# anguswilliams91/bpl-next

Hardware: NVIDIA B200
Metric: logdensity_grad_match_evals_per_s (higher is better)
Workload: dtype f32

## Files before the change

bpl_next_b200/csrc/api.cu:

```cuda
#include <limits.h>
#include <stdarg.h>
#include <stdlib.h>
#include <string.h>

#include <algorithm>
#include <atomic>
#include <mutex>
#include <new>

#include "common.cuh"
#include "plan.h"
#include "problem.h"
#include "loo.h"
#include "score_grid.h"
#include "simulate.h"

namespace bplx {

static thread_local char g_err[1024] = "";
static std::atomic<unsigned long long> g_launches{0};

void set_error(const char* fmt, ...) {
  va_list ap;
  va_start(ap, fmt);
// ... 59 lines not shown
    }
#pragma unroll
  for (int s = 0; s < 4; s++)
#pragma unroll
    for (int k = 0; k < 4; k++) tile[s][threadIdx.y + 8 * k][threadIdx.x] = v[s][k];
  __syncthreads();
#pragma unroll
  for (int s = 0; s < 4; s++)
#pragma unroll
    for (int k = 0; k < 4; k++) {
      const int c = c0 + threadIdx.y + 8 * k, r = r0 + s * 32 + threadIdx.x;
      if (r < R && c < Cc) out[(size_t)c * ldo + r] = tile[s][threadIdx.x][threadIdx.y + 8 * k];
    }
}
static int launch_transpose(const float* in, float* out, int R, int Cc, size_t ldi, size_t ldo, cudaStream_t s) {
  const dim3 grid((unsigned)((Cc + 31) / 32), (unsigned)((R + 127) / 128));
  BPLX_REQUIRE(grid.y <= 65535u, BPLX_E_UNSUPPORTED, "transpose of %d rows", R);
  transpose_kernel<<<grid, dim3(32, 8), 0, s>>>(in, out, R, Cc, ldi, ldo);
  BPLX_CUDA(cudaGetLastError());
  note_launch(1);
  return BPLX_OK;
}

static size_t align256(size_t n) { return (n + 255) / 256 * 256; }
static size_t transpose_room(const KernelParams& kp, int C) {
  if ((size_t)C * (size_t)kp.D < env_switches().transpose_min_elems) return 0;
  return 2 * (((size_t)C + 31) / 32 * 32) * (size_t)kp.D * sizeof(float);
}

static size_t workspace_bytes(const KernelParams& kp, int C) {
  const size_t Cpad = ((size_t)C + 31) / 32 * 32;
  if (kp.model == BPLX_DYNAMIC)
    return ((size_t)kp.G * kp.T * 2 + (kp.dyn_hyp_ws ? (size_t)kp.G * 16 : 0)) * Cpad * sizeof(float);
  if (kp.Cf <= 0) return 0;
  return (size_t)kp.V * Cpad * sizeof(float);
}

static int enqueue(const bplx_problem* p, int C, int layout, int ld, const float* theta, float* lp, float* grad,
                   float* corr_coef, void* ws, size_t ws_bytes, cudaStream_t stream, bool pdl = false, bool lik = false) {
  BPLX_REQUIRE(p != nullptr, BPLX_E_INVALID, "problem is NULL");
  BPLX_REQUIRE(C > 0, BPLX_E_INVALID, "num_chains must be positive (got %d)", C);
  BPLX_REQUIRE(theta && lp && grad, BPLX_E_INVALID, "theta, lp and grad must not be NULL");
  if (layout == BPLX_CHAIN_MAJOR && !env_switches().no_transpose) {
    const size_t base = align256(workspace_bytes(p->kp, C)), room = transpose_room(p->kp, C);
    if (room > 0 && ws != nullptr && ws_bytes >= base + room) {
      const int Dc = lik ? p->lik_D : p->kp.D;
      const size_t ldm = ld > 0 ? (size_t)ld : (size_t)Dc, Cpad = ((size_t)C + 31) / 32 * 32;
      BPLX_REQUIRE(ldm >= (size_t)Dc, BPLX_E_INVALID, "chain-major ld (%d) < D (%d)", ld, Dc);
      float* tin = reinterpret_cast<float*>(static_cast<char*>(ws) + base);
      float* tout = tin + Cpad * (size_t)p->kp.D;
      int rc = launch_transpose(theta, tin, C, Dc, ldm, Cpad, stream);
      if (rc != BPLX_OK) return rc;
      rc = enqueue(p, C, BPLX_CHAIN_MINOR, (int)Cpad, tin, lp, tout, corr_coef, ws, base, stream, pdl, lik);
      if (rc != BPLX_OK) return rc;
      return launch_transpose(tout, grad, Dc, C, Cpad, ldm, stream);
    }
  }
  KernelParams kp = p->kp;
  if (lik) {
    BPLX_REQUIRE(kp.model != BPLX_DYNAMIC, BPLX_E_UNSUPPORTED, "bplx_loglik_fwdbwd: DYNAMIC is not supported");
    kp.lik_only = 1;
    kp.off = p->lik_off;
    for (int i = 0; i < 12; i++) kp.hyper[i] = p->lik_hyper[i];
    kp.nhyper = p->lik_nhyper;
    kp.D = p->lik_D;
    kp.K = 0;
    kp.const_term = p->lik_const;
  }
// ... 7 lines not shown
    BPLX_REQUIRE(kp.sd >= C, BPLX_E_INVALID, "chain-minor ld (%d) < num_chains (%d)", ld, C);
  } else {
    BPLX_REQUIRE(false, BPLX_E_INVALID, "unknown layout %d", layout);
  }
  BPLX_REQUIRE((long long)kp.D * (long long)kp.sd + (long long)C * (long long)kp.sc < (1ll << 31), BPLX_E_UNSUPPORTED,
               "theta / grad of %d x %d elements exceed the 31-bit element index of the kernel", C, kp.D);
  const size_t need = workspace_bytes(kp, C);
  BPLX_REQUIRE(ws_bytes >= need && (need == 0 || ws != nullptr), BPLX_E_WORKSPACE,
               "workspace too small: %zu bytes given, %zu needed", ws_bytes, need);
  kp.C = C;
  kp.Cpad = (C + 31) / 32 * 32;
  kp.theta = theta;
  kp.lp = lp;
  kp.grad = grad;
  kp.corr_coef = corr_coef;
  kp.scratch = static_cast<float*>(ws);
  int si = 0;
  const int groups = (C + kChains - 1) / kChains;
  for (int i = kNumSplits - 1; i >= 1; i--)
    if (p->s1[i] && (1 << i) <= kp.split_hint && groups <= p->max_clusters[i]) {
      si = i;
      break;
    }
  if (const int want = env_switches().split) {
    for (int i = 0; i < kNumSplits; i++)
      if ((1 << i) == want && p->s1[i] && (i == 0 || p->max_clusters[i] > 0)) si = i;
  }
  auto use_split = [&](int i) {
    kp.split = 1 << i;
    kp.stream1 = p->s1[i];
    kp.stream2 = p->s2[i];
    kp.warp_b1 = p->wb1[i];
    kp.warp_b2 = p->wb2[i];
  };
  use_split(si);
  kp.group0 = 0;
  kp.ngroups = groups;
  if (kp.model == BPLX_DYNAMIC) return launch_logdensity_dynamic(kp, stream);
  int ti = 0;
  const int rest = p->sm_count > 0 ? groups % p->sm_count : 0;
  if (si == 0 && rest > 0 && rest < groups && !env_switches().split && !env_switches().no_tail_split) {
    for (int i = kNumSplits - 1; i >= 1; i--)
      if (p->s1[i] && (1 << i) <= kp.split_hint && rest <= p->max_clusters[i] && rest * (1 << i) <= p->sm_count) {
        ti = i;
        break;
      }
  }
  if (ti == 0) return launch_logdensity(kp, p->wb[si], stream, pdl);
  kp.ngroups = groups - rest;
  int rc = launch_logdensity(kp, p->wb[0], stream, pdl);
  if (rc != BPLX_OK) return rc;
  use_split(ti);
  kp.group0 = groups - rest;
  kp.ngroups = rest;
  return launch_logdensity(kp, p->wb[ti], stream, pdl);
}

}

using namespace bplx;

extern "C" {

int bplx_problem_create(const bplx_problem_desc* desc, bplx_problem** out) {
  BPLX_REQUIRE(desc && out, BPLX_E_INVALID, "desc / out is NULL");
  *out = nullptr;
  HostPlan hp;
  std::string err;
  int rc = build_plan(*desc, &hp, &err);
  if (rc != BPLX_OK) {
    set_error("%s", err.c_str());
    return rc;
  }
  bplx_problem* p = new (std::nothrow) bplx_problem();
  BPLX_REQUIRE(p, BPLX_E_NOMEM, "out of host memory");
  auto fail = [&](int code) {
    bplx_problem_destroy(p);
    return code;
  };
  if (cudaGetDevice(&p->device) != cudaSuccess) {
    set_error("cudaGetDevice failed: no usable CUDA device (bplx has no CPU fallback)");
    return fail(BPLX_E_CUDA);
  }
  p->kp = hp.kp;
  p->layout = hp.layout;
  p->lik_off = hp.lik_off;
  for (int i = 0; i < 12; i++) p->lik_hyper[i] = hp.lik_hyper[i];
  p->lik_nhyper = hp.lik_nhyper;
  p->lik_D = hp.lik_D;
  p->lik_const = hp.lik_const;
  p->lik_layout = hp.lik_layout;
  KernelParams& kp = p->kp;
#define UP(vec, ptr)                                 \
  if ((rc = upload(p, hp.vec, &(ptr))) != BPLX_OK) return fail(rc)
  UP(stream1, p->s1[0]);
  UP(stream2, p->s2[0]);
  UP(warp_b1, p->wb1[0]);
  UP(warp_b2, p->wb2[0]);
  for (int i = 1; i < kNumSplits; i++) {
    if (hp.more[i - 1].stream1.empty()) continue;
    UP(more[i - 1].stream1, p->s1[i]);
    UP(more[i - 1].stream2, p->s2[i]);
    UP(more[i - 1].warp_b1, p->wb1[i]);
    UP(more[i - 1].warp_b2, p->wb2[i]);
  }
  auto keep_bounds = [&](int i, const std::vector<uint32_t>& b1, const std::vector<uint32_t>& b2) {
    const size_t cap = sizeof(p->wb[i].b1) / sizeof(uint32_t);
    for (size_t k = 0; k < b1.size() && k < cap; k++) p->wb[i].b1[k] = b1[k];
    for (size_t k = 0; k < b2.size() && k < cap; k++) p->wb[i].b2[k] = b2[k];
  };
  keep_bounds(0, hp.warp_b1, hp.warp_b2);
  for (int i = 1; i < kNumSplits; i++) keep_bounds(i, hp.more[i - 1].warp_b1, hp.more[i - 1].warp_b2);
  kp.stream1 = p->s1[0];
  kp.stream2 = p->s2[0];
  kp.warp_b1 = p->wb1[0];
  kp.warp_b2 = p->wb2[0];
  kp.split = 1;
  UP(team_vptr, kp.team_vptr);
  UP(team_flags, kp.team_flags);
  UP(v_team, kp.v_team);
  UP(v_conf, kp.v_conf);
  UP(conf_vptr, kp.conf_vptr);
  UP(conf_vlist, kp.conf_vlist);
  UP(yexp, kp.yexp);
  UP(yteam, kp.yteam);
  UP(yconf, kp.yconf);
  UP(Xs, kp.Xs);
  UP(gw_tptr, kp.gw_tptr);
  UP(gw_tlist, kp.gw_tlist);
#undef UP
  rc = kp.model == BPLX_DYNAMIC ? logdensity_dynamic_set_attributes() : logdensity_set_attributes(kp);
  if (rc != BPLX_OK) return fail(rc);
  if (cudaDeviceGetAttribute(&p->sm_count, cudaDevAttrMultiProcessorCount, p->device) != cudaSuccess) p->sm_count = 0;
  p->max_clusters[0] = 1 << 30;
  if (kp.model != BPLX_DYNAMIC)
    for (int i = 1; i < kNumSplits; i++) p->max_clusters[i] = p->s1[i] ? logdensity_max_clusters(kp, 1 << i) : 0;
  p->stats[0] = desc->num_matches;
  p->stats[1] = hp.n1;
  p->stats[2] = hp.n1_padded;
  p->stats[3] = hp.n2;
  p->stats[4] = hp.n2_padded;
  p->stats[5] = kp.smem_total;
  p->stats[6] = kp.nwarps;
  p->stats[7] = kp.V;
  if (kp.model != BPLX_DYNAMIC) {
    p->warp_stats.assign((size_t)kp.nwarps * 12, 0);
    for (int phase = 0; phase < 2; phase++) {
      const std::vector<unsigned char>& S = phase ? hp.stream2 : hp.stream1;
      const std::vector<uint32_t>& wb = phase ? hp.warp_b2 : hp.warp_b1;
      const size_t esz = (phase == 0 && kp.clip) ? sizeof(EntryClip) : sizeof(Entry);
      const uint32_t minp = phase ? kp.min_piece2 : kp.min_piece1;
      for (int w = 0; w < kp.nwarps && w + 1 < (int)wb.size(); w++) {
        long long* o = &p->warp_stats[(size_t)w * 12 + phase * 6];
        const uint32_t len = wb[w + 1] - wb[w];
        o[5] = (len + kp.stage_bytes - 1) / kp.stage_bytes;
        for (uint32_t st = 0; st < len; st += kp.stage_bytes) {
// ... 783 lines not shown
```

bpl_next_b200/csrc/k1_common.cuh:

```cuda
#pragma once
#include <float.h>

#include "common.cuh"
#include "plan.h"

namespace bplx {

namespace {


constexpr float kLn2 = 0.693147180559945309f;
constexpr unsigned kFull = 0xffffffffu;

struct Hyp {
  float mu_d, sig_a, sig_d, mu[4], sig[4];
};

struct Lane {
  const float* th;
  float* gr;
  float* sc;
  int sd;
  bool active;
  __device__ __forceinline__ float ld(int d) const { return __ldg(th + (uint32_t)(d * sd)); }
// ... 71 lines not shown
  if (kind == kH1) {
    g[eAh1] += gx; g[eBh1] += gy;
  } else if (kind == kA1) {
    g[eBa1] += gx; g[eAa1] += gy;
  } else {
    g[eB0] += gx; g[eA0] += gy;
  }
}

template <bool ADD>
__device__ __forceinline__ void put_raw(const KernelParams& kp, const Lane& ln, int t, const float (&g)[6], float& hacc) {
  const ThetaOffsets& o = kp.off;
  const float ra = g[eAh1] + g[eAa1] + g[eA0];
  const float rd = -(g[eBh1] + g[eBa1] + g[eB0]);
  const float rx[4] = {g[eAh1], g[eAa1], -g[eBh1], -g[eBa1]};
  if (kp.ndec == 0) hacc += rx[0];
  if (!ln.active) return;
  if (ADD) {
    red_add(ln.g(o.za + t), ra);
    red_add(ln.g(o.zd + t), rd);
  } else {
    *ln.g(o.za + t) = ra;
    *ln.g(o.zd + t) = rd;
  }
#pragma unroll
  for (int i = 0; i < 4; i++) {
    if (i < kp.ndec) {
      if (ADD) red_add(ln.g(o.dec[i] + t), rx[i]);
      else *ln.g(o.dec[i] + t) = rx[i];
    }
  }
}

__device__ __forceinline__ void put_side(const KernelParams& kp, float* q, const float (&g)[6], float& hacc) {
  q[0] = g[eAh1] + g[eAa1] + g[eA0];
  q[32] = -(g[eBh1] + g[eBa1] + g[eB0]);
  const float rx[4] = {g[eAh1], g[eAa1], -g[eBh1], -g[eBa1]};
  if (kp.ndec == 0) hacc += rx[0];
#pragma unroll
  for (int i = 0; i < 4; i++)
    if (i < kp.ndec) q[(2 + i) * 32] = rx[i];
}

struct Ring {
  uint32_t ring, bar;
  uint32_t S;
  const unsigned char* src;
  uint32_t total;
  uint32_t gs0, gs_next;
  int lane;

  __device__ __forceinline__ void init(uint32_t ring_, uint32_t bar_, uint32_t S_, int lane_) {
    ring = ring_; bar = bar_; S = S_; lane = lane_;
    total = gs0 = gs_next = 0;
    src = nullptr;
    if (lane == 0) {
#pragma unroll
      for (int s = 0; s < kStages; s++) mbar_init(bar + 8 * s, 1);
      fence_mbar_init();
      fence_proxy_async();
    }
    __syncwarp();
  }
  __device__ __forceinline__ void issue(uint32_t k) {
    const uint32_t b0 = k * S;
    if (lane == 0 && b0 < total) {
      const uint32_t bytes = min(S, total - b0);
      const uint32_t slot = (gs0 + k) % kStages;
      mbar_arrive_expect_tx(bar + 8 * slot, bytes);
      tma_load_1d(ring + slot * S, src + b0, bytes, bar + 8 * slot);
    }
  }
  __device__ __forceinline__ void begin(const void* src_, uint32_t total_bytes) {
    __syncwarp();
// ... 140 lines not shown
```

bpl_next_b200/csrc/logdensity.cu:

```cuda
#include <cooperative_groups.h>

#include <math.h>

#include "k1_common.cuh"
#include "problem.h"

namespace cg = cooperative_groups;

#ifdef BPLX_TIMELINE
__device__ unsigned long long g_timeline[32 * 24];
#define BPLX_STAMP(i)                                                                    \
  do {                                                                                   \
    if (blockIdx.x == 0 && (threadIdx.x & 31) == 0) {                                    \
      unsigned long long t_;                                                             \
      asm volatile("mov.u64 %0, %%globaltimer;" : "=l"(t_));                             \
      g_timeline[(threadIdx.x >> 5) * 24 + (i)] = t_;                                    \
    }                                                                                    \
  } while (0)
#define BPLX_STAMP_DEP(i, dep)                                                           \
  do {                                                                                   \
    if (blockIdx.x == 0 && (threadIdx.x & 31) == 0) {                                    \
      unsigned long long t_;                                                             \
      asm volatile("mov.u64 %0, %%globaltimer;" : "=l"(t_) : "f"(dep));                  \
      g_timeline[(threadIdx.x >> 5) * 24 + (i)] = t_;                                    \
// ... 397 lines not shown
  BPLX_STAMP(5);
  float gc = 0.0f;
  {
    float g[6] = {0.0f, 0.0f, 0.0f, 0.0f, 0.0f, 0.0f}, cacc = 0.0f;
    const uint32_t nst = ring.num_stages();
    for (uint32_t k = 0; k < nst; k++) {
      uint32_t bytes;
      const uint32_t a0 = ring.acquire(k, &bytes);
      if (k == 0) BPLX_STAMP(18);
      uint32_t a = a0;
      const uint32_t aend = a0 + bytes;
      while (a + kp.min_piece2 <= aend) {
        const Hdr L = unpack_hdr(lds128u(a));
        a += 16;
        if (L.flags & kTeamFirst) {
#pragma unroll
          for (int e = 0; e < 6; e++) g[e] = 0.0f;
        }
        float2 own = lds64(tab + L.own_off);
        if (L.kind >= kH0) { const float s = own.x; own.x = own.y; own.y = s; }
        const bool home = (L.kind & 1) == 0;
        float lt, du, gx, gy;
        if (!CLIP) tau_piece<kTauPlain>(a, L, own, home, cc, tab, lt, du, gx, gy);
        else if (noclip) tau_piece<kTauUnclipped>(a, L, own, home, cc, tab, lt, du, gx, gy);
        else tau_piece<kTauClipped>(a, L, own, home, cc, tab, lt, du, gx, gy);
        if (home) {
          lp_acc = fmaf(lt, kLn2, lp_acc);
          gc += du;
        }
        add_own(g, L.kind, gx, gy);
        if (kp.Cf > 0) {
          cacc += L.kind == kH1 ? gx - gy : gy - gx;
          if (L.flags & kVteamLast) {
            if (ln.active) red_add(ln.sc + (size_t)L.vteam * kp.Cpad, cacc);
            cacc = 0.0f;
          }
        }
        if (L.flags & kTeamLast) {
          if (p2s) put_side(kp, p2_tab + (((L.kind & 1) * kp.T + L.team) * (2 + ndec)) * 32 + lane, g, hacc);
          else put_raw<true>(kp, ln, (int)L.team, g, hacc);
        }
      }
      ring.release(k);
    }
  }
  BPLX_STAMP(6);
  red_gc[warp * 32 + lane] = gc;
  __syncthreads();
  gc = 0.0f;
  for (int w = 0; w < W; w++) gc += red_gc[w * 32 + lane];
  if (S > 1) {
    if (warp == 0) dsm_st_f32(a_cl + (uint32_t)(crank * 32 + lane) * 4u, gc);
    cg::this_cluster().sync();
    gc = 0.0f;
    for (int q = 0; q < S; q++) gc += dsm_ld_f32(a_cl + (uint32_t)(q * 32 + lane) * 4u);
  }
  {
    const float t11 = fmaxf(1.0f - cc, 0.0f);
    gc -= kp.w11 / t11;
    if (vwarp == 0 && kp.w11 != 0.0f) lp_acc = fmaf(kp.w11, logf(t11), lp_acc);
  }

  BPLX_STAMP(7);
  Fixup fx;
  fx.h1 = 0u;
  fx.confs = 0u;
#pragma unroll
  for (int which = 0; which < 2; which++) {
    const uint32_t packed = dsm_ld_u32(a_found + (uint32_t)(which * 32 + lane) * 4u);
    fx.teams[which] = 0xffffffffu;
    fx.vts[which] = 0xffffffffu;
    fx.vx[which] = fx.vy[which] = 0.0f;
// ... 10 lines not shown
        fx.vy[0] = (qlam == 1 && yfree) ? wgt : 0.0f;
      } else {
        const float wgt = -gc * r / best[2];
        fx.vx[1] = xfree ? wgt : 0.0f;
        fx.vy[1] = yfree ? wgt : 0.0f;
      }
      fx.h1 |= (h1 ? 1u : 0u) << which;
      fx.vts[which] = own_v | (opp_v << 16);
      if (kp.Cf > 0)
        fx.confs |= ((uint32_t)__ldg(kp.v_conf + own_v) | ((uint32_t)__ldg(kp.v_conf + opp_v) << 8)) << (16 * which);
    }
  }

  BPLX_STAMP(8);
  const bool has_rho = !dc && !lik;
  const float pri = lik ? 0.0f : 1.0f;
  float u = 0.5f, rho = 0.0f, inv_s2 = 1.0f;
  if (has_rho) {
    u = red_hyp[11 * 32 + lane];
    rho = 2.0f * u - 1.0f;
    inv_s2 = 1.0f / (1.0f - rho * rho);
  }
  float a_mu_d = 0.0f, a_ls_a = 0.0f, a_ls_d = 0.0f, a_rho = 0.0f, a_mu[4], a_ls[4];
#pragma unroll
  for (int i = 0; i < 4; i++) a_mu[i] = a_ls[i] = 0.0f;
  {
    Hyp hy;
    hy.mu_d = red_hyp[0 * 32 + lane]; hy.sig_a = red_hyp[1 * 32 + lane]; hy.sig_d = red_hyp[2 * 32 + lane];
#pragma unroll
    for (int i = 0; i < 4; i++) { hy.mu[i] = red_hyp[(3 + i) * 32 + lane]; hy.sig[i] = red_hyp[(7 + i) * 32 + lane]; }

    for (int t = vwarp; t < kp.T; t += VW) {
      const float za = ln.ld(o.za + t), zd = ln.ld(o.zd + t);
      const uint32_t v0 = (uint32_t)__ldg(kp.team_vptr + t), nv = (uint32_t)__ldg(kp.team_vptr + t + 1) - v0;
      const float4 ys = __ldg(reinterpret_cast<const float4*>(kp.yteam + (size_t)t * 8));
      const float2 ys2 = __ldg(reinterpret_cast<const float2*>(kp.yteam + (size_t)t * 8 + 4));
      float ra = ld_cg(ln.g(o.za + t)) + ys.x;
      float rd = ld_cg(ln.g(o.zd + t)) + ys.y;
      float rx[4] = {ys.z, ys.w, ys2.x, ys2.y};
      float dec[4] = {0.0f, 0.0f, 0.0f, 0.0f};
#pragma unroll
      for (int i = 0; i < 4; i++) {
        if (i < ndec) {
          dec[i] = ln.ld(o.dec[i] + t);
          rx[i] += ld_cg(ln.g(o.dec[i] + t));
        }
      }
      if (p2s) {
#pragma unroll
        for (int side = 0; side < 2; side++) {
          const float* q = p2_tab + ((side * kp.T + t) * (2 + ndec)) * 32 + lane;
          ra += q[0];
          rd += q[32];
#pragma unroll
          for (int i = 0; i < 4; i++)
            if (i < ndec) rx[i] += q[(2 + i) * 32];
        }
      }
#pragma unroll
      for (int which = 0; which < 2; which++) {
        if ((fx.vts[which] & 0xffffu) - v0 < nv) fold_fixup(fx, which, 0, ra, rd, rx);
        if ((fx.vts[which] >> 16) - v0 < nv) fold_fixup(fx, which, 1, ra, rd, rx);
      }
      float p_za, p_zd;
      if (has_rho) {
        const float e = zd - rho * za;
        const float es = e * inv_s2;
        lp_acc -= 0.5f * (za * za + e * es);
        p_za = -za + rho * es;
        p_zd = -es;
        a_rho += es * za - rho * es * es + rho * inv_s2;
      } else {
        lp_acc -= pri * 0.5f * (za * za + zd * zd);
        p_za = -pri * za;
        p_zd = -pri * zd;
      }
      if (ln.active) {
        *ln.g(o.za + t) = fmaf(hy.sig_a, ra, p_za);
        *ln.g(o.zd + t) = fmaf(hy.sig_d, rd, p_zd);
      }
      a_ls_a = fmaf(hy.sig_a * za, ra, a_ls_a);
      a_ls_d = fmaf(hy.sig_d * zd, rd, a_ls_d);
      a_mu_d += rd;
      if (dc) a_mu[0] += rx[0];
#pragma unroll
      for (int i = 0; i < 4; i++) {
        if (i < ndec) {
          lp_acc -= pri * 0.5f * dec[i] * dec[i];
          if (ln.active) *ln.g(o.dec[i] + t) = fmaf(hy.sig[i], rx[i], -pri * dec[i]);
          a_mu[i] += rx[i];
          a_ls[i] = fmaf(hy.sig[i] * dec[i], rx[i], a_ls[i]);
        }
      }
      if (kp.K > 0) {
        dsm_st_f32(a_teamrows + (uint32_t)(t * 64 + lane) * 4u, ra);
        dsm_st_f32(a_teamrows + (uint32_t)(t * 64 + 32 + lane) * 4u, rd);
      }
    }
    if (dc) a_mu[0] += hacc;
  }
  for (int k = vwarp; k < kp.Cf; k += VW) {
    const float cf = ln.ld(o.conf + k);
    float s = __ldg(kp.yconf + k) - pri * cf;
    lp_acc -= pri * 0.5f * cf * cf;
    const int j0 = __ldg(kp.conf_vptr + k), j1 = __ldg(kp.conf_vptr + k + 1);
    for (int j = j0; j < j1; j++) s += ld_cg(ln.sc + (size_t)__ldg(kp.conf_vlist + j) * kp.Cpad);
#pragma unroll
    for (int ws = 0; ws < 4; ws++)
      if (fx.vts[ws >> 1] != 0xffffffffu && ((fx.confs >> (8 * ((ws >> 1) * 2 + (ws & 1)))) & 0xffu) == (uint32_t)k)
        s += fixup_conf(fx, ws >> 1, ws & 1);
    if (ln.active) *ln.g(o.conf + k) = s;
  }

  BPLX_STAMP(9);
  float* part = reinterpret_cast<float*>(smem + kp.epi_part);
  {
    float* p = part + (size_t)warp * kPartRows * 32 + lane;
    p[0 * 32] = lp_acc; p[1 * 32] = a_mu_d; p[2 * 32] = a_ls_a; p[3 * 32] = a_ls_d;
#pragma unroll
    for (int i = 0; i < 4; i++) { p[(4 + i) * 32] = a_mu[i]; p[(8 + i) * 32] = a_ls[i]; }
    p[12 * 32] = a_rho;
  }
  __syncthreads();
  if (S > 1) {
    for (int row = warp; row < kAccRows; row += W) {
      float s = 0.0f;
      for (int w = 0; w < W; w++) s += part[((size_t)w * kPartRows + row) * 32 + lane];
      dsm_st_f32(a_partcl + (uint32_t)((crank * kPartRows + row) * 32 + lane) * 4u, s);
    }
    cg::this_cluster().sync();
    if (crank != 0) return;
  }
  BPLX_STAMP(10);
  auto total = [&](int row) {
    float s = 0.0f;
    if (S > 1) {
      for (int q = 0; q < S; q++) s += dsm_ld_f32(a_partcl + (uint32_t)((q * kPartRows + row) * 32 + lane) * 4u);
    } else {
      for (int w = 0; w < W; w++) s += part[((size_t)w * kPartRows + row) * 32 + lane];
// ... 129 lines not shown
```

bpl_next_b200/csrc/plan.cc:

```cpp
#include "plan.h"

#include <algorithm>
#include <cmath>
#include <cstdarg>
#include <cstdio>
#include <cstdlib>
#include <cstring>
#include <map>
#include <numeric>

namespace bplx {
namespace {

struct RawEntry {
  uint32_t opp;
  uint8_t cls;
  double w, wyx, wyy;
};

std::string fmt(const char* f, ...) {
  char buf[512];
  va_list ap;
  va_start(ap, f);
  vsnprintf(buf, sizeof buf, f, ap);
  va_end(ap);
  return buf;
}

void add_site(std::string* s, const char* name, int off, int count, const char* tr) {
  *s += fmt("%s:%d:%d:%s;", name, off, count, tr);
}

int make_layout(int model, int T, int K, int Cf, ThetaOffsets* o, std::string* s) {
  ThetaOffsets z;
  memset(&z, 0xff, sizeof z);
  int d = 0;
  auto scalar = [&](const char* n, const char* tr) { add_site(s, n, d, 1, tr); return d++; };
  auto vec = [&](const char* n, int cnt, const char* tr) {
    add_site(s, n, d, cnt, tr);
    int r = d;
    d += cnt;
    return r;
// ... 284 lines not shown
    for (size_t i = 0; i < yc.size(); i++) P.yconf[i] = (float)yc[i];
  }
  P.Xs.assign(d.covariates ? d.covariates : nullptr, d.covariates ? d.covariates + (size_t)T * K : nullptr);

  auto own_off = [&](int v, int kind) -> uint32_t {
    uint32_t base = kind == kH1 ? kp.tabP1 : kind == kA1 ? kp.tabQ1 : kp.tabP0;
    return base + (uint32_t)v * kRowBytes;
  };
  auto opp_base = [&](int kind) -> uint32_t { return kind == kH1 ? kp.tabQ1 : kind == kA1 ? kp.tabP1 : kp.tabP0; };

  auto merge = [](std::vector<RawEntry>& v) {
    std::stable_sort(v.begin(), v.end(), [](const RawEntry& a, const RawEntry& b) {
      return a.cls != b.cls ? a.cls < b.cls : a.opp < b.opp;
    });
    size_t o = 0;
    for (size_t i = 0; i < v.size(); i++) {
      if (o && v[o - 1].cls == v[i].cls && v[o - 1].opp == v[i].opp) {
        v[o - 1].w += v[i].w;
        v[o - 1].wyx += v[i].wyx;
        v[o - 1].wyy += v[i].wyy;
      } else {
        v[o++] = v[i];
      }
    }
    v.resize(o);
  };
  for (auto& v : raw1) merge(v);
  for (auto& v : raw2) merge(v);
  P.team_flags.assign(T, 0);
  for (int v = 0; v < V; v++)
    for (int k = 0; k < 4; k++)
      if (!raw1[(size_t)v * 4 + k].empty()) P.team_flags[P.v_team[v]] |= 1;

  auto team_costs = [&](const std::vector<std::vector<RawEntry>>& raw, double per_entry, double per_list,
                        double per_team) {
    std::vector<double> cost(T, 0.0);
    for (int v = 0; v < V; v++)
      for (int k = 0; k < 4; k++) {
        const size_t n = raw[(size_t)v * 4 + k].size();
        if (n) cost[P.v_team[v]] += per_list * (1.0 + (double)n / 100.0) + per_entry * (double)n;
      }
    for (int t = 0; t < T; t++)
      if (cost[t] > 0.0) cost[t] += per_team;
    return cost;
  };
  auto assign = [&](const std::vector<double>& cost, int W, std::vector<std::vector<int>>* teams) {
    std::vector<int> order(T);
    std::iota(order.begin(), order.end(), 0);
    std::stable_sort(order.begin(), order.end(), [&](int a, int b) { return cost[a] > cost[b]; });
    std::vector<double> load(W, 0.0);
    teams->assign(W, {});
    for (int t : order) {
      if (cost[t] == 0.0) continue;
      int best = 0;
      for (int w = 1; w < W; w++)
        if (load[w] < load[best]) best = w;
      load[best] += cost[t];
      (*teams)[best].push_back(t);
    }
    for (auto& v : *teams) std::sort(v.begin(), v.end());
    return *std::max_element(load.begin(), load.end());
  };
  const std::vector<double> cost1 = team_costs(raw1, kp.clip ? 16.0 : 6.0, 40.0, 30.0);
  const std::vector<double> cost2 = team_costs(raw2, 12.0, 60.0, 30.0);
  auto smem_need = [&](int W, uint32_t stage) {
    const uint32_t epi = (K > 0 ? (uint32_t)T * kRowBytes : 0u) + (uint32_t)(W + kMaxSplit) * kPartRows * 128u;
    const uint32_t tabb = (std::max(table_bytes, epi) + 127u) / 128u * 128u;
    return tabb + (uint32_t)W * kStages * stage + 128u + (uint32_t)W * kStages * 8u + 3u * 256u + 2u * 128u + 2u * 128u +
           12u * 128u + (uint32_t)(W + kMaxSplit) * 128u;
  };
  const uint32_t kSmemMax = 227u * 1024u;
  int W = 0;
  uint32_t stage = 1024;
  std::vector<std::vector<int>> w1, w2;
  if (force_warps <= 0) {
    if (const char* e = getenv("BPLX_NWARPS")) force_warps = atoi(e);
  }
  if (const char* e = getenv("BPLX_STAGE")) stage = (uint32_t)atoi(e) == 512u ? 512u : 1024u;
  if (force_warps > 0) {
    W = std::max(1, std::min(force_warps, kMaxWarps));
    if (smem_need(W, stage) > kSmemMax) stage = 512;
  } else {
    double best = 0.0;
    for (int cand : {4, 8, 12, 16, 20, 24}) {
      if (cand > kMaxWarps) continue;
      uint32_t st = stage;
      if (smem_need(cand, st) > kSmemMax) st = 512;
      if (smem_need(cand, st) > kSmemMax) continue;
      std::vector<std::vector<int>> t1, t2;
      const double span = assign(cost1, cand, &t1) + assign(cost2, cand, &t2) + 4.0 * cand + (st == 512 ? 0.05 * best : 0.0);
      if (W == 0 || span < 0.97 * best) best = span, W = cand, stage = st;
    }
    if (W == 0) W = 4, stage = 512;
  }
  kp.nwarps = W;
  kp.stage_bytes = stage;
  kp.force_clip_forms = 0;
  if (const char* e = getenv("BPLX_CLIP_FORMS")) kp.force_clip_forms = atoi(e);
  {
    std::vector<std::vector<int>> t1, t2;
    const double span = assign(cost1, W, &t1) + assign(cost2, W, &t2);
    kp.split_hint = span >= 32000.0 ? 8 : span >= 16000.0 ? 4 : span >= 8000.0 ? 2 : 1;
  }

  std::vector<std::vector<int>> w2_items;
  kp.smem_p2 = 0;
  {
    std::vector<std::pair<int, double>> units;
    for (int t = 0; t < T; t++)
      for (int side = 0; side < 2; side++) {
        double c = 0.0;
        for (int v = P.team_vptr[t]; v < P.team_vptr[t + 1]; v++)
          for (int k = side; k < 4; k += 2) {
            const size_t n = raw2[(size_t)v * 4 + k].size();
            if (n) c += 60.0 * (1.0 + (double)n / 100.0) + 12.0 * (double)n;
          }
        if (c > 0.0) units.push_back({t * 4 + (1 << side), c + 30.0});
      }
    std::stable_sort(units.begin(), units.end(), [](const auto& a, const auto& b) { return a.second > b.second; });
    std::vector<double> load(W, 0.0);
    std::vector<std::vector<int>> items(W);
    for (const auto& u : units) {
      int best = 0;
      for (int w = 1; w < W; w++)
        if (load[w] < load[best]) best = w;
      load[best] += u.second;
      items[best].push_back(u.first);
    }
    for (auto& v : items) std::sort(v.begin(), v.end());
    std::vector<std::vector<int>> t2;
    const double span_team = assign(cost2, W, &t2);
    const double span_unit = units.empty() ? 0.0 : *std::max_element(load.begin(), load.end());
    const uint32_t p2_bytes = 2u * (uint32_t)T * (uint32_t)(2 + kp.ndec) * 128u;
    const bool off = getenv("BPLX_NO_P2SPLIT") != nullptr;
    if (!off && Cf <= 0 && span_unit < 0.85 * span_team && smem_need(W, stage) + p2_bytes <= kSmemMax) {
      w2_items = items;
      kp.smem_p2 = 1;
    }
  }

  const uint32_t zero_row = (uint32_t)V * kRowBytes;
  auto put = [](std::vector<unsigned char>* s, const void* p, size_t n) {
    const unsigned char* b = static_cast<const unsigned char*>(p);
    s->insert(s->end(), b, b + n);
  };
  auto emit = [&](int Wtot, std::vector<unsigned char>* s1, std::vector<unsigned char>* s2, std::vector<uint32_t>* wb1,
                  std::vector<uint32_t>* wb2) {
  const bool by_side = kp.smem_p2 != 0 && Wtot == kp.nwarps;
  const int W = Wtot;
  assign(cost1, W, &w1);
  assign(cost2, W, &w2);
  std::vector<std::vector<int>> it1(W), it2(W);
  for (int w = 0; w < W; w++) {
    for (int t : w1[w]) it1[w].push_back(t * 4 + 3);
    for (int t : w2[w]) it2[w].push_back(t * 4 + 3);
  }
  if (by_side) it2 = w2_items;
  P.n1 = P.n2 = P.n1_padded = P.n2_padded = P.nlists1 = P.nlists2 = 0;
  wb1->assign(W + 1, 0);
  wb2->assign(W + 1, 0);
  for (int phase = 1; phase <= 2; phase++) {
    const auto& raw = phase == 1 ? raw1 : raw2;
    const auto& by_warp = phase == 1 ? it1 : it2;
    std::vector<unsigned char>& S = phase == 1 ? *s1 : *s2;
    std::vector<uint32_t>& wb = phase == 1 ? *wb1 : *wb2;
    const size_t esz = (phase == 1 && kp.clip) ? sizeof(EntryClip) : sizeof(Entry);
    const size_t gran = 16;
    const size_t min_piece = sizeof(ListHdr) + gran;
    (phase == 1 ? kp.min_piece1 : kp.min_piece2) = (uint32_t)min_piece;
    S.clear();
    for (int w = 0; w < W; w++) {
      const size_t wstart = S.size();
      for (int item : by_warp[w]) {
        const int t = item >> 2, sides = item & 3;
        size_t team_first_hdr = (size_t)-1, last_hdr = 0;
        for (int v = P.team_vptr[t]; v < P.team_vptr[t + 1]; v++) {
          size_t vteam_last_hdr = (size_t)-1;
          for (int k = 0; k < 4; k++) {
            const auto& r = raw[(size_t)v * 4 + k];
            if (r.empty() || !((sides >> (k & 1)) & 1)) continue;
            (phase == 1 ? P.n1 : P.n2) += (long long)r.size();
            std::vector<unsigned char> body;
            std::vector<uint8_t> cls;
            if (phase == 1) {
              for (const RawEntry& e : r) {
                const uint32_t o = opp_base(k) + e.opp * kRowBytes;
                if (kp.clip) {
                  EntryClip x{o, (float)e.w, (float)e.wyx, (float)e.wyy};
                  put(&body, &x, sizeof x);
                } else {
                  Entry x{o, (float)e.w};
                  put(&body, &x, sizeof x);
                }
                cls.push_back(0);
              }
              while (!kp.clip && (cls.size() & 1)) {
                Entry x{opp_base(k) + zero_row, 0.0f};
                put(&body, &x, sizeof x);
                cls.push_back(0);
              }
            } else {
              size_t i = 0;
              for (int c = 0; c < 3; c++) {
                const uint32_t comp = c == 2 ? 4u : 0u;
                size_t cnt = 0;
                for (; i < r.size() && r[i].cls == c; i++, cnt++) {
                  Entry x{opp_base(k) + r[i].opp * kRowBytes + comp, (float)r[i].w};
                  put(&body, &x, sizeof x);
                  cls.push_back((uint8_t)c);
                }
                if (cnt & 1) {
                  Entry x{opp_base(k) + zero_row + comp, 0.0f};
                  put(&body, &x, sizeof x);
                  cls.push_back((uint8_t)c);
                }
              }
            }
            (phase == 1 ? P.n1_padded : P.n2_padded) += (long long)cls.size();
            size_t done = 0;
            while (done < cls.size()) {
              size_t in_stage = (S.size() - wstart) % stage;
              if (stage - in_stage < min_piece) {
                S.resize(S.size() + (stage - in_stage), 0);
                in_stage = 0;
              }
              const size_t space = stage - in_stage - sizeof(ListHdr);
              const size_t take = std::min(cls.size() - done, space / gran * gran / esz);
              ListHdr H{};
              H.own_off = own_off(v, k);
              H.vteam = (uint16_t)v;
              H.kind = (uint8_t)k;
              H.team = (uint16_t)t;
              uint16_t cnt[3] = {0, 0, 0};
              for (size_t i = done; i < done + take; i++) cnt[cls[i]]++;
              H.n0 = cnt[0];
              H.n1 = cnt[1];
              H.n2 = cnt[2];
              const size_t hdr_at = S.size();
              put(&S, &H, sizeof H);
              put(&S, body.data() + done * esz, take * esz);
              done += take;
              (phase == 1 ? P.nlists1 : P.nlists2)++;
              if (team_first_hdr == (size_t)-1) team_first_hdr = hdr_at;
              vteam_last_hdr = last_hdr = hdr_at;
            }
          }
          if (vteam_last_hdr != (size_t)-1) reinterpret_cast<ListHdr*>(&S[vteam_last_hdr])->flags |= kVteamLast;
        }
        if (team_first_hdr != (size_t)-1) {
          reinterpret_cast<ListHdr*>(&S[team_first_hdr])->flags |= kTeamFirst;
          reinterpret_cast<ListHdr*>(&S[last_hdr])->flags |= kTeamLast;
        }
      }
      wb[w + 1] = (uint32_t)S.size();
    }
    if (S.empty()) S.resize(16, 0);
  }
  };
  for (int i = kNumSplits - 1; i >= 1; i--)
    emit(W << i, &P.more[i - 1].stream1, &P.more[i - 1].stream2, &P.more[i - 1].warp_b1, &P.more[i - 1].warp_b2);
  emit(W, &P.stream1, &P.stream2, &P.warp_b1, &P.warp_b2);

  kp.epi_team = 0;
  kp.epi_part = K > 0 ? (uint32_t)T * kRowBytes : 0u;
  kp.epi_cl = kp.epi_part + (uint32_t)W * kPartRows * 128u;
  const uint32_t epi = kp.epi_cl + (uint32_t)kMaxSplit * kPartRows * 128u;
  kp.tab_bytes = (std::max(table_bytes, epi) + 127u) / 128u * 128u;
  kp.smem_ring = kp.tab_bytes;
  kp.smem_bar = kp.smem_ring + (uint32_t)W * kStages * stage;
  kp.smem_red = (kp.smem_bar + (uint32_t)W * kStages * 8u + 127u) / 128u * 128u;
  kp.smem_red_cl = kp.smem_red + 3u * 256u + 2u * 128u + 2u * 128u + 12u * 128u + (uint32_t)W * 128u;
  kp.smem_total = kp.smem_red_cl + (uint32_t)kMaxSplit * 128u;
  if (kp.smem_p2) {
    kp.smem_p2 = kp.smem_total;
    kp.smem_total += 2u * (uint32_t)T * (uint32_t)(2 + kp.ndec) * 128u;
  }
  if (kp.smem_total > kSmemMax)
    FAIL(BPLX_E_UNSUPPORTED, "problem needs %u bytes of shared memory per CTA (max %u): too many (team, confederation) pairs (%d)",
         kp.smem_total, kSmemMax, V);
#undef FAIL
  return BPLX_OK;
}

#include "plan_dynamic.inc"

}
```

bpl_next_b200/csrc/plan.h:

```cpp
#pragma once
#include <stdint.h>

#include <string>
#include <vector>

#include "../../include/bplx.h"

namespace bplx {

constexpr int kChains = 32;
constexpr int kRowBytes = 256;
constexpr int kMaxCov = 16;
constexpr int kMaxWarps = 24;
constexpr int kMaxWarpsDyn = 20;
constexpr int kStages = 2;
constexpr int kAccRows = 13;
constexpr int kPartRows = 16;
constexpr int kMaxSplit = 8;
constexpr int kNumSplits = 4;

enum Kind : uint8_t { kH1 = 0, kA1 = 1, kH0 = 2, kA0 = 3 };
enum Exponent : int { eAh1 = 0, eBh1 = 1, eBa1 = 2, eAa1 = 3, eA0 = 4, eB0 = 5 };

constexpr uint8_t kTeamFirst = 1;
constexpr uint8_t kTeamLast = 2;
constexpr uint8_t kVteamLast = 4;
constexpr uint8_t kGwFirst = 8;
constexpr uint8_t kStageEnd = 16;
constexpr uint8_t kPhase2 = 32;

struct Entry {
  uint32_t off;
  float w;
};
struct EntryClip {
  uint32_t off;
  float w;
  float wyx;
  float wyy;
};

struct ListHdr {
  uint32_t own_off;
  uint16_t vteam;
  uint8_t kind;
  uint8_t flags;
  uint16_t n0;
  uint16_t n1;
  uint16_t n2;
  uint16_t team;
};
static_assert(sizeof(ListHdr) == 16, "ListHdr must be 16 bytes");

struct ThetaOffsets {
  int mean_defence, log_std_attack, log_std_defence;
  int mean[4];
  int log_std[4];
  int u;
  int beta_a, beta_d;
  int za, zd;
  int dec[4];
  int conf;
// ... 14 lines not shown
struct KernelParams {
  int model, T, K, Cf, V;
  int G;
  int as_written;
  int D, nwarps;
  int ndec;
  int clip;
  int lik_only;
  int has1, has0;
  uint32_t tabP1, tabQ1, tabP0;
  uint32_t tab_bytes;
  uint32_t stage_bytes;
  uint32_t min_piece1, min_piece2;
  uint32_t smem_ring, smem_bar, smem_red, smem_total;
  uint32_t epi_team, epi_part;
  uint32_t epi_cl;
  uint32_t smem_red_cl;
  uint32_t smem_p2;
  uint32_t dyn_state, dyn_part, dyn_hyp, dyn_fin;
  int dyn_nbuf;
  int dyn_hyp_ws;
  int split_hint;
  int group0, ngroups;
  int force_clip_forms;
  ThetaOffsets off;
  const unsigned char* stream1;
  const unsigned char* stream2;
  const uint32_t* warp_b1;
  const uint32_t* warp_b2;
  const int32_t* team_vptr;
  const uint8_t* team_flags;
  const uint16_t* v_team;
  const uint8_t* v_conf;
  const int32_t* conf_vptr;
  const int32_t* conf_vlist;
  const float* yexp;
  const float* yteam;
  const float* yconf;
  const float* Xs;
  const int32_t* gw_tptr;
  const uint16_t* gw_tlist;
  HyperDesc hyper[12];
  int nhyper;
  float w11;
  float const_term;
  int C;
  int split;
  int sd, sc;
  const float* theta;
  float* lp;
  float* grad;
  float* corr_coef;
  float* scratch;
  int Cpad;
};

struct SplitStreams {
  std::vector<unsigned char> stream1, stream2;
  std::vector<uint32_t> warp_b1, warp_b2;
};

struct HostPlan {
  KernelParams kp{};
  ThetaOffsets lik_off{};
  HyperDesc lik_hyper[12]{};
  int lik_nhyper = 0, lik_D = 0;
  float lik_const = 0.0f;
  std::string lik_layout;
  std::vector<unsigned char> stream1, stream2;
  std::vector<uint32_t> warp_b1, warp_b2;
  SplitStreams more[kNumSplits - 1];
  std::vector<int32_t> team_vptr, conf_vptr, conf_vlist;
  std::vector<uint8_t> team_flags;
  std::vector<uint16_t> v_team;
  std::vector<uint8_t> v_conf;
  std::vector<float> yexp, yteam, yconf, Xs;
  std::vector<int32_t> gw_tptr;
  std::vector<uint16_t> gw_tlist;
  std::string layout;
  long long n1 = 0, n2 = 0, n1_padded = 0, n2_padded = 0, nlists1 = 0, nlists2 = 0;
};

int build_plan(const bplx_problem_desc& d, HostPlan* out, std::string* err, int force_warps = 0);

}
```

bpl_next_b200/csrc/problem.h:

```cpp
#pragma once
#include <mutex>
#include <string>
#include <vector>

#include "common.cuh"
#include "plan.h"

struct bplx_problem {
  int device = 0;
  bplx::KernelParams kp{};
  std::string layout;
  bplx::ThetaOffsets lik_off{};
  bplx::HyperDesc lik_hyper[12]{};
  int lik_nhyper = 0, lik_D = 0;
  float lik_const = 0.0f;
  std::string lik_layout;
  const unsigned char* s1[bplx::kNumSplits] = {};
  const unsigned char* s2[bplx::kNumSplits] = {};
  const uint32_t* wb1[bplx::kNumSplits] = {};
  const uint32_t* wb2[bplx::kNumSplits] = {};
  bplx::WarpBounds wb[bplx::kNumSplits] = {};
  int max_clusters[bplx::kNumSplits] = {0, 0, 0, 0};
  std::vector<void*> dev_allocs;
  std::mutex mu;
  int host_cap = 0;
  float *h_theta = nullptr, *h_out = nullptr;
  float *d_theta = nullptr, *d_out = nullptr;
  float *d_tin = nullptr, *d_tout = nullptr;
  int tr_cap = 0;
  void* d_ws = nullptr;
  size_t d_ws_bytes = 0;
  cudaStream_t host_stream = nullptr;
  cudaStream_t host_in = nullptr, host_out = nullptr;
  cudaEvent_t host_ev[48] = {};
  int sm_count = 0;
  long long stats[8] = {0, 0, 0, 0, 0, 0, 0, 0};
  std::vector<long long> warp_stats;
};

namespace bplx {
int launch_logdensity(const KernelParams& kp, const WarpBounds& wb, cudaStream_t stream, bool pdl);
int logdensity_set_attributes(const KernelParams& kp);
int logdensity_max_clusters(const KernelParams& kp, int split);
int launch_logdensity_dynamic(const KernelParams& kp, cudaStream_t stream);
int logdensity_dynamic_set_attributes();
}
```

Measured before the change: 846.0 billion.

## Split heavy teams' phase-2 work across warps by home/away side

After: 851.9 billion, median of 6. Within noise of the previous version (+0.7%).

```diff
diff --git a/bpl_next_b200/csrc/api.cu b/bpl_next_b200/csrc/api.cu
--- a/bpl_next_b200/csrc/api.cu
+++ b/bpl_next_b200/csrc/api.cu
@@ -115,8 +115,7 @@
   const size_t Cpad = ((size_t)C + 31) / 32 * 32;
   if (kp.model == BPLX_DYNAMIC)
     return ((size_t)kp.G * kp.T * 2 + (kp.dyn_hyp_ws ? (size_t)kp.G * 16 : 0)) * Cpad * sizeof(float);
-  if (kp.Cf <= 0) return 0;
-  return (size_t)kp.V * Cpad * sizeof(float);
+  return ((size_t)(kp.Cf > 0 ? kp.V : 0) + (size_t)kp.side_rows) * Cpad * sizeof(float);
 }
 
 static int enqueue(const bplx_problem* p, int C, int layout, int ld, const float* theta, float* lp, float* grad,
@@ -190,6 +189,7 @@
     kp.stream2 = p->s2[i];
     kp.warp_b1 = p->wb1[i];
     kp.warp_b2 = p->wb2[i];
+    kp.side = p->side[i];
   };
   use_split(si);
   kp.group0 = 0;
@@ -255,12 +255,14 @@
   UP(stream2, p->s2[0]);
   UP(warp_b1, p->wb1[0]);
   UP(warp_b2, p->wb2[0]);
+  UP(side, p->side[0]);
   for (int i = 1; i < kNumSplits; i++) {
     if (hp.more[i - 1].stream1.empty()) continue;
     UP(more[i - 1].stream1, p->s1[i]);
     UP(more[i - 1].stream2, p->s2[i]);
     UP(more[i - 1].warp_b1, p->wb1[i]);
     UP(more[i - 1].warp_b2, p->wb2[i]);
+    UP(more[i - 1].side, p->side[i]);
   }
   auto keep_bounds = [&](int i, const std::vector<uint32_t>& b1, const std::vector<uint32_t>& b2) {
     const size_t cap = sizeof(p->wb[i].b1) / sizeof(uint32_t);
@@ -273,13 +275,12 @@
   kp.stream2 = p->s2[0];
   kp.warp_b1 = p->wb1[0];
   kp.warp_b2 = p->wb2[0];
+  kp.side = p->side[0];
   kp.split = 1;
   UP(team_vptr, kp.team_vptr);
   UP(team_flags, kp.team_flags);
   UP(v_team, kp.v_team);
   UP(v_conf, kp.v_conf);
-  UP(conf_vptr, kp.conf_vptr);
-  UP(conf_vlist, kp.conf_vlist);
   UP(yexp, kp.yexp);
   UP(yteam, kp.yteam);
   UP(yconf, kp.yconf);
diff --git a/bpl_next_b200/csrc/k1_common.cuh b/bpl_next_b200/csrc/k1_common.cuh
--- a/bpl_next_b200/csrc/k1_common.cuh
+++ b/bpl_next_b200/csrc/k1_common.cuh
@@ -127,14 +127,19 @@
   }
 }
 
-__device__ __forceinline__ void put_side(const KernelParams& kp, float* q, const float (&g)[6], float& hacc) {
-  q[0] = g[eAh1] + g[eAa1] + g[eA0];
-  q[32] = -(g[eBh1] + g[eBa1] + g[eB0]);
+__device__ __forceinline__ void put_side(const KernelParams& kp, float* q, size_t stride, bool store, const float (&g)[6],
+                                         float& hacc) {
   const float rx[4] = {g[eAh1], g[eAa1], -g[eBh1], -g[eBa1]};
   if (kp.ndec == 0) hacc += rx[0];
+  if (!store) return;
+  q[0] = g[eAh1] + g[eAa1] + g[eA0];
+  q[stride] = -(g[eBh1] + g[eBa1] + g[eB0]);
 #pragma unroll
   for (int i = 0; i < 4; i++)
-    if (i < kp.ndec) q[(2 + i) * 32] = rx[i];
+    if (i < kp.ndec) q[(2 + i) * stride] = rx[i];
+}
+__device__ __forceinline__ size_t side_vrow(const KernelParams& kp, int base, uint32_t team, uint32_t v) {
+  return (size_t)(base + 2 + kp.ndec + (int)v - __ldg(kp.team_vptr + team));
 }
 
 struct Ring {
diff --git a/bpl_next_b200/csrc/logdensity.cu b/bpl_next_b200/csrc/logdensity.cu
--- a/bpl_next_b200/csrc/logdensity.cu
+++ b/bpl_next_b200/csrc/logdensity.cu
@@ -453,12 +453,18 @@
         if (kp.Cf > 0) {
           cacc += L.kind == kH1 ? gx - gy : gy - gx;
           if (L.flags & kVteamLast) {
-            if (ln.active) red_add(ln.sc + (size_t)L.vteam * kp.Cpad, cacc);
+            if (L.flags & kSidePart) {
+              if (ln.active) ln.sc[side_vrow(kp, __ldg(kp.side + L.team), L.team, L.vteam) * kp.Cpad] = cacc;
+            } else if (ln.active) {
+              red_add(ln.sc + (size_t)L.vteam * kp.Cpad, cacc);
+            }
             cacc = 0.0f;
           }
         }
         if (L.flags & kTeamLast) {
-          if (p2s) put_side(kp, p2_tab + (((L.kind & 1) * kp.T + L.team) * (2 + ndec)) * 32 + lane, g, hacc);
+          if (p2s) put_side(kp, p2_tab + (((L.kind & 1) * kp.T + L.team) * (2 + ndec)) * 32 + lane, 32, true, g, hacc);
+          else if (L.flags & kSidePart)
+            put_side(kp, ln.sc + (size_t)__ldg(kp.side + L.team) * kp.Cpad, kp.Cpad, ln.active, g, hacc);
           else put_raw<true>(kp, ln, (int)L.team, g, hacc);
         }
       }
@@ -535,6 +541,7 @@
 
     for (int t = vwarp; t < kp.T; t += VW) {
       const float za = ln.ld(o.za + t), zd = ln.ld(o.zd + t);
+      const int srow = __ldg(kp.side + t);
       const uint32_t v0 = (uint32_t)__ldg(kp.team_vptr + t), nv = (uint32_t)__ldg(kp.team_vptr + t + 1) - v0;
       const float4 ys = __ldg(reinterpret_cast<const float4*>(kp.yteam + (size_t)t * 8));
       const float2 ys2 = __ldg(reinterpret_cast<const float2*>(kp.yteam + (size_t)t * 8 + 4));
@@ -548,6 +555,14 @@
           dec[i] = ln.ld(o.dec[i] + t);
           rx[i] += ld_cg(ln.g(o.dec[i] + t));
         }
+      }
+      if (srow >= 0) {
+        const float* q = ln.sc + (size_t)srow * kp.Cpad;
+        ra += ld_cg(q);
+        rd += ld_cg(q + kp.Cpad);
+#pragma unroll
+        for (int i = 0; i < 4; i++)
+          if (i < ndec) rx[i] += ld_cg(q + (size_t)(2 + i) * kp.Cpad);
       }
       if (p2s) {
 #pragma unroll
@@ -606,8 +621,8 @@
     const float cf = ln.ld(o.conf + k);
     float s = __ldg(kp.yconf + k) - pri * cf;
     lp_acc -= pri * 0.5f * cf * cf;
-    const int j0 = __ldg(kp.conf_vptr + k), j1 = __ldg(kp.conf_vptr + k + 1);
-    for (int j = j0; j < j1; j++) s += ld_cg(ln.sc + (size_t)__ldg(kp.conf_vlist + j) * kp.Cpad);
+    const int j0 = __ldg(kp.side + kp.T + k), j1 = __ldg(kp.side + kp.T + k + 1);
+    for (int j = j0; j < j1; j++) s += ld_cg(ln.sc + (size_t)__ldg(kp.side + j) * kp.Cpad);
 #pragma unroll
     for (int ws = 0; ws < 4; ws++)
       if (fx.vts[ws >> 1] != 0xffffffffu && ((fx.confs >> (8 * ((ws >> 1) * 2 + (ws & 1)))) & 0xffu) == (uint32_t)k)
diff --git a/bpl_next_b200/csrc/plan.cc b/bpl_next_b200/csrc/plan.cc
--- a/bpl_next_b200/csrc/plan.cc
+++ b/bpl_next_b200/csrc/plan.cc
@@ -8,6 +8,7 @@
 #include <cstring>
 #include <map>
 #include <numeric>
+#include <queue>
 
 namespace bplx {
 namespace {
@@ -358,37 +359,94 @@
     for (int k = 0; k < 4; k++)
       if (!raw1[(size_t)v * 4 + k].empty()) P.team_flags[P.v_team[v]] |= 1;
 
-  auto team_costs = [&](const std::vector<std::vector<RawEntry>>& raw, double per_entry, double per_list,
-                        double per_team) {
-    std::vector<double> cost(T, 0.0);
-    for (int v = 0; v < V; v++)
+  struct PhaseCost {
+    std::vector<double> whole, side;
+    std::vector<char> can_split;
+  };
+  const bool team_deal = getenv("BPLX_TEAM_DEAL") != nullptr;
+  auto phase_cost = [&](const std::vector<std::vector<RawEntry>>& raw, const double (&per_entry)[2],
+                        const double (&per_list)[2], double per_team) {
+    PhaseCost pc;
+    pc.whole.assign(T, 0.0);
+    pc.side.assign((size_t)T * 2, 0.0);
+    pc.can_split.assign(T, !team_deal);
+    for (int v = 0; v < V; v++) {
+      const int t = P.v_team[v];
+      bool has[2] = {false, false};
       for (int k = 0; k < 4; k++) {
         const size_t n = raw[(size_t)v * 4 + k].size();
-        if (n) cost[P.v_team[v]] += per_list * (1.0 + (double)n / 100.0) + per_entry * (double)n;
-      }
-    for (int t = 0; t < T; t++)
-      if (cost[t] > 0.0) cost[t] += per_team;
-    return cost;
-  };
-  auto assign = [&](const std::vector<double>& cost, int W, std::vector<std::vector<int>>* teams) {
-    std::vector<int> order(T);
-    std::iota(order.begin(), order.end(), 0);
-    std::stable_sort(order.begin(), order.end(), [&](int a, int b) { return cost[a] > cost[b]; });
-    std::vector<double> load(W, 0.0);
-    teams->assign(W, {});
-    for (int t : order) {
-      if (cost[t] == 0.0) continue;
-      int best = 0;
-      for (int w = 1; w < W; w++)
-        if (load[w] < load[best]) best = w;
-      load[best] += cost[t];
-      (*teams)[best].push_back(t);
-    }
-    for (auto& v : *teams) std::sort(v.begin(), v.end());
-    return *std::max_element(load.begin(), load.end());
-  };
-  const std::vector<double> cost1 = team_costs(raw1, kp.clip ? 16.0 : 6.0, 40.0, 30.0);
-  const std::vector<double> cost2 = team_costs(raw2, 12.0, 60.0, 30.0);
+        if (!n) continue;
+        const double c = per_list[k & 1] * (1.0 + (double)n / 100.0) + per_entry[k & 1] * (double)n;
+        pc.whole[t] += c;
+        pc.side[(size_t)t * 2 + (k & 1)] += c;
+        has[k & 1] = true;
+      }
+      if (!has[0] || !has[1]) pc.can_split[t] = 0;
+    }
+    for (int t = 0; t < T; t++) {
+      if (pc.whole[t] > 0.0) pc.whole[t] += per_team;
+      for (int s = 0; s < 2; s++)
+        if (pc.side[(size_t)t * 2 + s] > 0.0) pc.side[(size_t)t * 2 + s] += per_team;
+    }
+    return pc;
+  };
+  auto lpt = [&](const PhaseCost& pc, const std::vector<int>& cand, int k, int W, std::vector<std::vector<int>>* items) {
+    std::vector<char> split(T, 0);
+    for (int i = 0; i < k; i++) split[cand[i]] = 1;
+    std::vector<std::pair<int, double>> units;
+    for (int t = 0; t < T; t++) {
+      if (pc.whole[t] == 0.0) continue;
+      if (split[t]) {
+        units.push_back({t * 4 + 1, pc.side[(size_t)t * 2]});
+        units.push_back({t * 4 + 2, pc.side[(size_t)t * 2 + 1]});
+      } else {
+        units.push_back({t * 4 + 3, pc.whole[t]});
+      }
+    }
+    std::stable_sort(units.begin(), units.end(), [](const auto& a, const auto& b) { return a.second > b.second; });
+    std::priority_queue<std::pair<double, int>, std::vector<std::pair<double, int>>, std::greater<>> q;
+    for (int w = 0; w < W; w++) q.push({0.0, w});
+    if (items) items->assign(W, {});
+    double span = 0.0;
+    for (const auto& u : units) {
+      auto [load, w] = q.top();
+      q.pop();
+      load += u.second;
+      span = std::max(span, load);
+      q.push({load, w});
+      if (items) (*items)[w].push_back(u.first);
+    }
+    if (items)
+      for (auto& v : *items) {
+        std::sort(v.begin(), v.end());
+        size_t o = 0;
+        for (size_t i = 0; i < v.size(); i++) {
+          if (o && v[o - 1] + 1 == v[i] && (v[i] & 3) == 2) v[o - 1] |= 3;
+          else v[o++] = v[i];
+        }
+        v.resize(o);
+      }
+    return span;
+  };
+  auto deal = [&](const PhaseCost& pc, int W, bool allow_split, std::vector<std::vector<int>>* items) {
+    std::vector<int> cand;
+    if (allow_split)
+      for (int t = 0; t < T; t++)
+        if (pc.can_split[t]) cand.push_back(t);
+    std::stable_sort(cand.begin(), cand.end(), [&](int a, int b) { return pc.whole[a] < pc.whole[b]; });
+    const double span0 = lpt(pc, cand, 0, W, nullptr);
+    double best = span0;
+    int bk = 0;
+    for (int k = 1; k <= std::min((int)cand.size(), 2 * W); k++) {
+      const double s = lpt(pc, cand, k, W, nullptr);
+      if (s < best) best = s, bk = k;
+    }
+    if (best >= 0.99 * span0) bk = 0;
+    return bk == 0 && !items ? span0 : lpt(pc, cand, bk, W, items);
+  };
+  const double e1 = kp.clip ? 16.0 : 6.0;
+  const PhaseCost cost1 = phase_cost(raw1, {e1, e1}, {40.0, 40.0}, 30.0);
+  const PhaseCost cost2 = phase_cost(raw2, {12.9, 11.1}, {60.0, 60.0}, 30.0);
   auto smem_need = [&](int W, uint32_t stage) {
     const uint32_t epi = (K > 0 ? (uint32_t)T * kRowBytes : 0u) + (uint32_t)(W + kMaxSplit) * kPartRows * 128u;
     const uint32_t tabb = (std::max(table_bytes, epi) + 127u) / 128u * 128u;
@@ -398,7 +456,6 @@
   const uint32_t kSmemMax = 227u * 1024u;
   int W = 0;
   uint32_t stage = 1024;
-  std::vector<std::vector<int>> w1, w2;
   if (force_warps <= 0) {
     if (const char* e = getenv("BPLX_NWARPS")) force_warps = atoi(e);
   }
@@ -413,8 +470,8 @@
       uint32_t st = stage;
       if (smem_need(cand, st) > kSmemMax) st = 512;
       if (smem_need(cand, st) > kSmemMax) continue;
-      std::vector<std::vector<int>> t1, t2;
-      const double span = assign(cost1, cand, &t1) + assign(cost2, cand, &t2) + 4.0 * cand + (st == 512 ? 0.05 * best : 0.0);
+      const double span = deal(cost1, cand, false, nullptr) + deal(cost2, cand, false, nullptr) + 4.0 * cand +
+                          (st == 512 ? 0.05 * best : 0.0);
       if (W == 0 || span < 0.97 * best) best = span, W = cand, stage = st;
     }
     if (W == 0) W = 4, stage = 512;
@@ -424,8 +481,7 @@
   kp.force_clip_forms = 0;
   if (const char* e = getenv("BPLX_CLIP_FORMS")) kp.force_clip_forms = atoi(e);
   {
-    std::vector<std::vector<int>> t1, t2;
-    const double span = assign(cost1, W, &t1) + assign(cost2, W, &t2);
+    const double span = deal(cost1, W, false, nullptr) + deal(cost2, W, false, nullptr);
     kp.split_hint = span >= 32000.0 ? 8 : span >= 16000.0 ? 4 : span >= 8000.0 ? 2 : 1;
   }
 
@@ -454,8 +510,7 @@
       items[best].push_back(u.first);
     }
     for (auto& v : items) std::sort(v.begin(), v.end());
-    std::vector<std::vector<int>> t2;
-    const double span_team = assign(cost2, W, &t2);
+    const double span_team = deal(cost2, W, false, nullptr);
     const double span_unit = units.empty() ? 0.0 : *std::max_element(load.begin(), load.end());
     const uint32_t p2_bytes = 2u * (uint32_t)T * (uint32_t)(2 + kp.ndec) * 128u;
     const bool off = getenv("BPLX_NO_P2SPLIT") != nullptr;
@@ -470,26 +525,25 @@
     const unsigned char* b = static_cast<const unsigned char*>(p);
     s->insert(s->end(), b, b + n);
   };
-  auto emit = [&](int Wtot, std::vector<unsigned char>* s1, std::vector<unsigned char>* s2, std::vector<uint32_t>* wb1,
-                  std::vector<uint32_t>* wb2) {
+  kp.side_rows = 0;
+  auto emit = [&](int Wtot, SplitStreams* out) {
+  std::vector<unsigned char>* s1 = &out->stream1;
+  std::vector<unsigned char>* s2 = &out->stream2;
   const bool by_side = kp.smem_p2 != 0 && Wtot == kp.nwarps;
   const int W = Wtot;
-  assign(cost1, W, &w1);
-  assign(cost2, W, &w2);
-  std::vector<std::vector<int>> it1(W), it2(W);
-  for (int w = 0; w < W; w++) {
-    for (int t : w1[w]) it1[w].push_back(t * 4 + 3);
-    for (int t : w2[w]) it2[w].push_back(t * 4 + 3);
-  }
+  std::vector<std::vector<int>> it1, it2;
+  deal(cost1, W, false, &it1);
   if (by_side) it2 = w2_items;
+  else deal(cost2, W, true, &it2);
+  std::vector<char> away_part(T, 0);
   P.n1 = P.n2 = P.n1_padded = P.n2_padded = P.nlists1 = P.nlists2 = 0;
-  wb1->assign(W + 1, 0);
-  wb2->assign(W + 1, 0);
+  out->warp_b1.assign(W + 1, 0);
+  out->warp_b2.assign(W + 1, 0);
   for (int phase = 1; phase <= 2; phase++) {
     const auto& raw = phase == 1 ? raw1 : raw2;
     const auto& by_warp = phase == 1 ? it1 : it2;
     std::vector<unsigned char>& S = phase == 1 ? *s1 : *s2;
-    std::vector<uint32_t>& wb = phase == 1 ? *wb1 : *wb2;
+    std::vector<uint32_t>& wb = phase == 1 ? out->warp_b1 : out->warp_b2;
     const size_t esz = (phase == 1 && kp.clip) ? sizeof(EntryClip) : sizeof(Entry);
     const size_t gran = 16;
     const size_t min_piece = sizeof(ListHdr) + gran;
@@ -499,6 +553,8 @@
       const size_t wstart = S.size();
       for (int item : by_warp[w]) {
         const int t = item >> 2, sides = item & 3;
+        const uint8_t part_flag = sides == 2 && !by_side ? kSidePart : 0;
+        if (part_flag) away_part[t] = 1;
         size_t team_first_hdr = (size_t)-1, last_hdr = 0;
         for (int v = P.team_vptr[t]; v < P.team_vptr[t + 1]; v++) {
           size_t vteam_last_hdr = (size_t)-1;
@@ -557,6 +613,7 @@
               H.vteam = (uint16_t)v;
               H.kind = (uint8_t)k;
               H.team = (uint16_t)t;
+              H.flags = part_flag;
               uint16_t cnt[3] = {0, 0, 0};
               for (size_t i = done; i < done + take; i++) cnt[cls[i]]++;
               H.n0 = cnt[0];
@@ -582,10 +639,39 @@
     }
     if (S.empty()) S.resize(16, 0);
   }
-  };
-  for (int i = kNumSplits - 1; i >= 1; i--)
-    emit(W << i, &P.more[i - 1].stream1, &P.more[i - 1].stream2, &P.more[i - 1].warp_b1, &P.more[i - 1].warp_b2);
-  emit(W, &P.stream1, &P.stream2, &P.warp_b1, &P.warp_b2);
+  std::vector<int32_t>& side = out->side;
+  side.assign(T, -1);
+  int rows = 0;
+  for (int t = 0; t < T; t++) {
+    if (!away_part[t]) continue;
+    side[t] = (Cf > 0 ? V : 0) + rows;
+    rows += 2 + kp.ndec + (Cf > 0 ? P.team_vptr[t + 1] - P.team_vptr[t] : 0);
+  }
+  kp.side_rows = std::max(kp.side_rows, rows);
+  if (Cf > 0) {
+    const size_t ptr0 = side.size();
+    side.resize(ptr0 + Cf + 1);
+    for (int c = 0; c < Cf; c++) {
+      side[ptr0 + c] = (int32_t)side.size();
+      for (int j = P.conf_vptr[c]; j < P.conf_vptr[c + 1]; j++) side.push_back(P.conf_vlist[j]);
+      for (int j = P.conf_vptr[c]; j < P.conf_vptr[c + 1]; j++) {
+        const int v = P.conf_vlist[j], t = P.v_team[v];
+        if (side[t] >= 0) side.push_back(side[t] + 2 + kp.ndec + (v - P.team_vptr[t]));
+      }
+    }
+    side[ptr0 + Cf] = (int32_t)side.size();
+  }
+  };
+  for (int i = kNumSplits - 1; i >= 1; i--) emit(W << i, &P.more[i - 1]);
+  {
+    SplitStreams one;
+    emit(W, &one);
+    P.stream1 = std::move(one.stream1);
+    P.stream2 = std::move(one.stream2);
+    P.warp_b1 = std::move(one.warp_b1);
+    P.warp_b2 = std::move(one.warp_b2);
+    P.side = std::move(one.side);
+  }
 
   kp.epi_team = 0;
   kp.epi_part = K > 0 ? (uint32_t)T * kRowBytes : 0u;
diff --git a/bpl_next_b200/csrc/plan.h b/bpl_next_b200/csrc/plan.h
--- a/bpl_next_b200/csrc/plan.h
+++ b/bpl_next_b200/csrc/plan.h
@@ -28,6 +28,7 @@
 constexpr uint8_t kGwFirst = 8;
 constexpr uint8_t kStageEnd = 16;
 constexpr uint8_t kPhase2 = 32;
+constexpr uint8_t kSidePart = 64;
 
 struct Entry {
   uint32_t off;
@@ -108,8 +109,6 @@
   const uint8_t* team_flags;
   const uint16_t* v_team;
   const uint8_t* v_conf;
-  const int32_t* conf_vptr;
-  const int32_t* conf_vlist;
   const float* yexp;
   const float* yteam;
   const float* yconf;
@@ -127,6 +126,8 @@
   float* lp;
   float* grad;
   float* corr_coef;
+  const int32_t* side;
+  int side_rows;
   float* scratch;
   int Cpad;
 };
@@ -134,6 +135,7 @@
 struct SplitStreams {
   std::vector<unsigned char> stream1, stream2;
   std::vector<uint32_t> warp_b1, warp_b2;
+  std::vector<int32_t> side;
 };
 
 struct HostPlan {
@@ -145,6 +147,7 @@
   std::string lik_layout;
   std::vector<unsigned char> stream1, stream2;
   std::vector<uint32_t> warp_b1, warp_b2;
+  std::vector<int32_t> side;
   SplitStreams more[kNumSplits - 1];
   std::vector<int32_t> team_vptr, conf_vptr, conf_vlist;
   std::vector<uint8_t> team_flags;
diff --git a/bpl_next_b200/csrc/problem.h b/bpl_next_b200/csrc/problem.h
--- a/bpl_next_b200/csrc/problem.h
+++ b/bpl_next_b200/csrc/problem.h
@@ -19,6 +19,7 @@
   const unsigned char* s2[bplx::kNumSplits] = {};
   const uint32_t* wb1[bplx::kNumSplits] = {};
   const uint32_t* wb2[bplx::kNumSplits] = {};
+  const int32_t* side[bplx::kNumSplits] = {};
   bplx::WarpBounds wb[bplx::kNumSplits] = {};
   int max_clusters[bplx::kNumSplits] = {0, 0, 0, 0};
   std::vector<void*> dev_allocs;
```
